# Ulixes-8/UNet-Implementations

Hardware: AMD Instinct MI355X
Metric: images/sec (512x512, bs/GPU=8) Our_UNet train step (higher is better)
Workload: dtype f32

## Files before the change

### unet-implementations_amd/csrc/conv_wino.hip

```cpp
#include "conv_params.h"
#include "lds_asm.h"
#include <utility>

namespace unet_conv {
namespace {

typedef int i32x4v __attribute__((ext_vector_type(4)));
template <int I> using wn_ic = std::integral_constant<int, I>;
template <int B, int... I, typename F>
__device__ __forceinline__ void wn_for_impl(std::integer_sequence<int, I...>, F&& f) {
  (f(wn_ic<B + I>{}), ...);
}
template <int B, int E, typename F>
__device__ __forceinline__ void wn_for(F&& f) {
  wn_for_impl<B>(std::make_integer_sequence<int, E - B>{}, f);
}

constexpr int WN_TH = 8, WN_TW = 32;
constexpr int WN_PW = WN_TW + 2, WN_PH = WN_TH + 2;
constexpr int WN_PPIX = WN_PH * WN_PW;
constexpr int WN_BN = 64;
constexpr int WN_KC = 8;
constexpr int WN_RP = 360;
constexpr int WN_BUF = 16 * 64 * WN_KC;
constexpr size_t WN_LDS = (size_t)(4 * WN_BUF + 2 * WN_KC * WN_RP) * sizeof(float);

__host__ __device__ __forceinline__ int wn_swz(int row, int k) {
  return 2 * ((k >> 1) ^ ((row >> 2) & 3)) + (k & 1);
}

struct WinoParams {
  IgemmParams g;
  const float* wu;
};

template <bool ACT, bool STATS, bool BSTATS, bool UP = false>
__global__ __launch_bounds__(512, 2) void conv_wino_kernel(const WinoParams wp) {
  const IgemmParams& p = wp.g;
  extern __shared__ __attribute__((aligned(16))) float smem[];
  float* Vs = smem;
  float* Us = smem + 2 * WN_BUF;
  float* Rs = smem + 4 * WN_BUF;

  const int tid = threadIdx.x, lane = tid & 63, wave = tid >> 6;
  const int H = p.Hin, W = p.Win;
  const int tiles_n = p.Ncols / WN_BN, tiles_x = W / WN_TW, tiles_y = H / WN_TH;
  int bid = xcd_remap(blockIdx.x, gridDim.x);
  const int tn = bid % tiles_n; bid /= tiles_n;
  const int tx = bid % tiles_x; bid /= tiles_x;
  const int ty = bid % tiles_y;
  const int n = bid / tiles_y;
  const int y0 = ty * WN_TH, x0 = tx * WN_TW, n0 = tn * WN_BN;
  const int Ktot = p.C0 + p.C1;
  const int chunks = Ktot / WN_KC;

  const __amdgpu_buffer_rsrc_t rs0 = __builtin_amdgcn_make_buffer_rsrc(
      const_cast<float*>(p.src0), 0, (int)p.src0_bytes, 0x00020000);
  const __amdgpu_buffer_rsrc_t rs1 = __builtin_amdgcn_make_buffer_rsrc(
      const_cast<float*>(p.src1 ? p.src1 : p.src0), 0, (int)p.src1_bytes, 0x00020000);

  const int half = tid & 1;
  unsigned voff0[UP ? 1 : 2], voff1[2];
  bool okslot[2];
#pragma unroll
  for (int i = 0; i < 2; ++i) {
    const int slot = tid + 512 * i;
    const int pix = slot >> 1;
    const int prow = pix / WN_PW, pcol = pix - prow * WN_PW;
    const int iy = y0 - 1 + prow, ix = x0 - 1 + pcol;
    const bool ok = slot < 2 * WN_PPIX && (unsigned)iy < (unsigned)H && (unsigned)ix < (unsigned)W;
    const unsigned lin = (unsigned)((n * H + iy) * W + ix);
    okslot[i] = ok;
    if (!UP) voff0[i] = ok ? (lin * (unsigned)p.C0 + half * 4) * 4u : 0x80000000u;
    voff1[i] = ok ? (lin * (unsigned)p.C1 + half * 4) * 4u : 0x80000000u;
  }
  int l_lin[2], l_meta[2];
  const int lw = W >> 1;
  if (UP) {
    const int h = H >> 1, w = W >> 1;
#pragma unroll
    for (int i = 0; i < 2; ++i) {
      const int slot = tid + 512 * i;
      const int pix = slot < 2 * WN_PPIX ? slot >> 1 : 0;
      const int prow = pix / WN_PW, pcol = pix - prow * WN_PW;
      int gy0 = (y0 >> 1) - 1 + (prow >> 1), gx0 = (x0 >> 1) - 1 + (pcol >> 1);
      int gy1 = gy0 + 1, gx1 = gx0 + 1;
      gy0 = gy0 < 0 ? 0 : (gy0 > h - 1 ? h - 1 : gy0);
      gy1 = gy1 < 0 ? 0 : (gy1 > h - 1 ? h - 1 : gy1);
      gx0 = gx0 < 0 ? 0 : (gx0 > w - 1 ? w - 1 : gx0);
      gx1 = gx1 < 0 ? 0 : (gx1 > w - 1 ? w - 1 : gx1);
      l_lin[i] = (n * h + gy0) * w + gx0;
      l_meta[i] = (gx1 - gx0) | ((gy1 - gy0) << 1) | ((pcol & 1) << 2) | ((prow & 1) << 3);
    }
  }
  constexpr int NSET = UP ? 1 : 2;
  f32x4 pr[NSET][2];
  f32x4 pt[UP ? 2 : 1][3];
  bool pup = false;
  f32x4 ca[NSET], cb[NSET];
#pragma unroll
  for (int q = 0; q < NSET; ++q) { ca[q] = f32x4{1.f, 1.f, 1.f, 1.f}; cb[q] = f32x4{0.f, 0.f, 0.f, 0.f}; }
  const unsigned hoff = (unsigned)half * 16u;
  auto load_raw = [&](int chunk, auto ic, auto setc) {
    constexpr int i = decltype(ic)::value;
    constexpr int Q = decltype(setc)::value;
    const int c = chunk * WN_KC;
    const bool first = c < p.C0;
    const __amdgpu_buffer_rsrc_t rs = first ? rs0 : rs1;
    const int Cs = first ? p.C0 : p.C1;
    const int cc = first ? c : c - p.C0;
    if (UP && first) {
      if (i == 1) pup = true;
      const unsigned o = (unsigned)(l_lin[i] * Cs + cc + half * 4);
      const unsigned dx = (l_meta[i] & 1) ? (unsigned)Cs : 0u;
      const unsigned dy = (l_meta[i] & 2) ? (unsigned)(lw * Cs) : 0u;
      pr[Q][i] = buf_ld4<float>(rs, o, 0u);
      if constexpr (UP) {
        pt[i][0] = buf_ld4<float>(rs, o + dx, 0u);
        pt[i][1] = buf_ld4<float>(rs, o + dy, 0u);
        pt[i][2] = buf_ld4<float>(rs, o + dy + dx, 0u);
      }
    } else {
      if (UP && i == 1) pup = false;
      unsigned vo = voff1[i];
      if constexpr (!UP) vo = first ? voff0[i] : voff1[i];
      pr[Q][i] = __builtin_bit_cast(f32x4, __builtin_amdgcn_raw_buffer_load_b128(rs, vo, cc * 4, 0));
    }
    if (ACT && i == 1) {
      const float* al = (first ? p.act0_alpha : p.act1_alpha) + ((size_t)n * Cs + cc);
      const float* be = (first ? p.act0_beta : p.act1_beta) + ((size_t)n * Cs + cc);
      ca[Q] = *reinterpret_cast<const f32x4*>(reinterpret_cast<const char*>(al) + hoff);
      cb[Q] = *reinterpret_cast<const f32x4*>(reinterpret_cast<const char*>(be) + hoff);
    }
  };
  const int rpix1 = tid < 2 * WN_PPIX - 512 ? 256 + (tid >> 1) : WN_PPIX + (tid & 15);
  float* const rdst0 = Rs + (half * 4) * WN_RP + (tid >> 1);
  float* const rdst1 = Rs + (half * 4) * WN_RP + rpix1;
  constexpr int RB = WN_KC * WN_RP;
#pragma unroll
  for (int i = 0; i < 2; ++i)
    if (!okslot[i] && tid + 512 * i < 2 * WN_PPIX) {
      float* d = i == 0 ? rdst0 : rdst1;
#pragma unroll
      for (int k = 0; k < 4; ++k) d[k * WN_RP] = d[RB + k * WN_RP] = 0.f;
    }
  auto store_raw = [&](auto ic, auto bc, auto setc) {
    constexpr int i = decltype(ic)::value;
    constexpr int B = decltype(bc)::value;
    constexpr int Q = decltype(setc)::value;
    f32x4 v = pr[Q][i];
    if (ACT) {
      const f32x4 a1 = ca[Q], b1 = cb[Q];
      const float sl = p.slope;
      bool done = false;
      if constexpr (UP) {
        if (pup) {
          const f32x4 p00 = act4f(v, a1, b1, sl, 1.f), p01 = act4f(pt[i][0], a1, b1, sl, 1.f);
          const f32x4 p10 = act4f(pt[i][1], a1, b1, sl, 1.f);
          const f32x4 p11 = act4f(pt[i][2], a1, b1, sl, 1.f);
          const float wx1 = (l_meta[i] & 4) ? 0.75f : 0.25f, wx0 = 1.f - wx1;
          const float wy1 = (l_meta[i] & 8) ? 0.75f : 0.25f, wy0 = 1.f - wy1;
          v = (p00 * wx0 + p01 * wx1) * wy0 + (p10 * wx0 + p11 * wx1) * wy1;
          done = true;
        }
      }
      if (!done) v = act4f(v, a1, b1, sl, 1.f);
    }
    if (okslot[i]) {
      float* d = (i == 0 ? rdst0 : rdst1) + B * RB;
      d[0] = v[0]; d[WN_RP] = v[1]; d[2 * WN_RP] = v[2]; d[3 * WN_RP] = v[3];
    }
  };
  const int t_tile = tid >> 3, t_ch = tid & 7;
  const unsigned t_ra = lds_addr(Rs + t_ch * WN_RP + (2 * (t_tile >> 4)) * WN_PW + 2 * (t_tile & 15));
  float* const t_vdst = Vs + t_tile * 8 + wn_swz(t_tile, t_ch);
  f32x2v tr[4];
  auto t_rd = [&](auto ac, auto bc) {
    constexpr int a = decltype(ac)::value;
    constexpr int B = decltype(bc)::value;
    constexpr int r0 = a == 0 ? 0 : (a == 1 ? 1 : (a == 2 ? 2 : 1));
    constexpr int r1 = a == 0 ? 2 : (a == 1 ? 2 : (a == 2 ? 1 : 3));
    tr[0] = lds_rd64<(B * RB + r0 * WN_PW) * 4>(t_ra);
    tr[1] = lds_rd64<(B * RB + r0 * WN_PW) * 4 + 8>(t_ra);
    tr[2] = lds_rd64<(B * RB + r1 * WN_PW) * 4>(t_ra);
    tr[3] = lds_rd64<(B * RB + r1 * WN_PW) * 4 + 8>(t_ra);
  };
  auto t_wr = [&](auto ac, auto bc) {
    constexpr int a = decltype(ac)::value;
    constexpr int B = decltype(bc)::value;
    lds_wait<15>(tr[0], tr[1], tr[2], tr[3]);
    const f32x2v lo = a == 1 ? tr[0] + tr[2] : tr[0] - tr[2];
    const f32x2v hi = a == 1 ? tr[1] + tr[3] : tr[1] - tr[3];
    float* Vb = t_vdst + B * WN_BUF;
    Vb[(4 * a + 0) * 512] = lo[0] - hi[0];
    Vb[(4 * a + 1) * 512] = lo[1] + hi[0];
    Vb[(4 * a + 2) * 512] = hi[0] - lo[1];
    Vb[(4 * a + 3) * 512] = lo[1] - hi[1];
  };
  const float* ubase = wp.wu + (size_t)((p.n_off / WN_BN + tn) * chunks) * WN_BUF;
  const int uwave = __builtin_amdgcn_readfirstlane(wave) * 1024;
  const unsigned lane16 = (unsigned)lane * 16u;
  const unsigned u_m0 = __builtin_amdgcn_readfirstlane(lds_addr(Us + uwave));
  auto dma_u = [&](int chunk, auto bc, auto ic) {
    constexpr int i = decltype(ic)::value;
    constexpr int B = decltype(bc)::value;
    const float* src = ubase + (size_t)chunk * WN_BUF + uwave;
    const unsigned m0v = u_m0 + B * WN_BUF * 4;
    dma16_sbase<i * 1024>(m0v, lane16, src);
  };

  const int tg = wave & 3, nh = wave >> 2;
  const int fm = lane & 15, fk = lane >> 4;
  const int fsw = 2 * (fk ^ ((fm >> 2) & 3));
  const unsigned va = lds_addr(Vs + (16 * tg + fm) * 8 + fsw);
  const unsigned ub = lds_addr(Us + (32 * nh + fm) * 8 + fsw);
  f32x4 acc[16][2];
#pragma unroll
  for (int x = 0; x < 16; ++x)
#pragma unroll
    for (int b = 0; b < 2; ++b) acc[x][b] = f32x4{0.f, 0.f, 0.f, 0.f};
  constexpr int FS = UP ? 1 : 2;
  f32x2v fa[FS], fb0[FS], fb1[FS];
  auto frag = [&](auto bc, auto xc) {
    constexpr int x = decltype(xc)::value;
    constexpr int B = decltype(bc)::value;
    constexpr int sl = x % FS;
    fa[sl] = lds_rd64<(B * WN_BUF + x * 512) * 4>(va);
    fb0[sl] = lds_rd64<(B * WN_BUF + x * 512) * 4>(ub);
    fb1[sl] = lds_rd64<(B * WN_BUF + x * 512 + 128) * 4>(ub);
  };
  auto mm = [&](auto xc) {
    constexpr int x = decltype(xc)::value;
    constexpr int sl = x % FS;
    acc[x][0] = __builtin_amdgcn_mfma_f32_16x16x4f32(fa[sl][0], fb0[sl][0], acc[x][0], 0, 0, 0);
    acc[x][1] = __builtin_amdgcn_mfma_f32_16x16x4f32(fa[sl][0], fb1[sl][0], acc[x][1], 0, 0, 0);
    acc[x][0] = __builtin_amdgcn_mfma_f32_16x16x4f32(fa[sl][1], fb0[sl][1], acc[x][0], 0, 0, 0);
    acc[x][1] = __builtin_amdgcn_mfma_f32_16x16x4f32(fa[sl][1], fb1[sl][1], acc[x][1], 0, 0, 0);
  };
  auto stage = [&](auto bc, auto xc, auto trc) {
    constexpr int x = decltype(xc)::value;
    constexpr int TR = decltype(trc)::value;
    constexpr int sl = x % FS;
    if constexpr (FS == 2) {
      if constexpr (x + 1 < 16) frag(bc, wn_ic<x + 1>{});
      lds_wait<(x + 1 < 16 ? 3 : 0) + TR>(fa[sl], fb0[sl], fb1[sl]);
      __builtin_amdgcn_sched_barrier(0);
      mm(xc);
    } else {
      lds_wait<0>(fa[sl], fb0[sl], fb1[sl]);
      __builtin_amdgcn_sched_barrier(0);
      mm(xc);
      if constexpr (x + 1 < 16) frag(bc, wn_ic<x + 1>{});
    }
  };

  using S0 = wn_ic<0>;
  using S1 = wn_ic<NSET - 1>;
  auto cl = [&](int c) { return c < chunks ? c : chunks - 1; };
  auto vm_done = [&]() {
    asm volatile("s_waitcnt vmcnt(0)" ::: "memory");
#pragma unroll
    for (int q = 0; q < NSET; ++q) reg_anchor(ca[q], cb[q]);
  };
  if constexpr (NSET == 2) {
    load_raw(0, wn_ic<0>{}, S0{});
    load_raw(0, wn_ic<1>{}, S0{});
    load_raw(cl(1), wn_ic<0>{}, S1{});
    load_raw(cl(1), wn_ic<1>{}, S1{});
    wn_for<0, 4>([&](auto ic) { dma_u(0, wn_ic<0>{}, ic); });
    vm_done();
    store_raw(wn_ic<0>{}, wn_ic<0>{}, S0{});
    store_raw(wn_ic<1>{}, wn_ic<0>{}, S0{});
    store_raw(wn_ic<0>{}, wn_ic<1>{}, S1{});
    store_raw(wn_ic<1>{}, wn_ic<1>{}, S1{});
    load_raw(cl(2), wn_ic<0>{}, S0{});
    load_raw(cl(2), wn_ic<1>{}, S0{});
    load_raw(cl(3), wn_ic<0>{}, S1{});
    load_raw(cl(3), wn_ic<1>{}, S1{});
    __syncthreads();
    wn_for<0, 4>([&](auto ac) {
      t_rd(ac, wn_ic<0>{});
      asm volatile("s_waitcnt lgkmcnt(0)" ::: "memory");
      t_wr(ac, wn_ic<0>{});
    });
  } else {
    load_raw(0, wn_ic<0>{}, S0{});
    load_raw(0, wn_ic<1>{}, S0{});
    wn_for<0, 4>([&](auto ic) { dma_u(0, wn_ic<0>{}, ic); });
    vm_done();
    store_raw(wn_ic<0>{}, wn_ic<0>{}, S0{});
    store_raw(wn_ic<1>{}, wn_ic<0>{}, S0{});
    load_raw(cl(1), wn_ic<0>{}, S0{});
    load_raw(cl(1), wn_ic<1>{}, S0{});
    __syncthreads();
    wn_for<0, 4>([&](auto ac) {
      t_rd(ac, wn_ic<0>{});
      asm volatile("s_waitcnt lgkmcnt(0)" ::: "memory");
      t_wr(ac, wn_ic<0>{});
    });
    vm_done();
    store_raw(wn_ic<0>{}, wn_ic<1>{}, S0{});
    store_raw(wn_ic<1>{}, wn_ic<1>{}, S0{});
    load_raw(cl(2), wn_ic<0>{}, S0{});
    load_raw(cl(2), wn_ic<1>{}, S0{});
  }
  auto chunk_body = [&](int c, auto bc) {
    constexpr int B = decltype(bc)::value;
    using NB = wn_ic<B ^ 1>;
    using SB = wn_ic<(NSET == 2 ? B : 0)>;
    if constexpr (NSET == 2) {
      if constexpr (ACT) asm volatile("s_waitcnt vmcnt(4) lgkmcnt(0)" ::: "memory");
      else asm volatile("s_waitcnt vmcnt(2) lgkmcnt(0)" ::: "memory");
    } else {
      asm volatile("s_waitcnt vmcnt(0) lgkmcnt(0)" ::: "memory");
    }
    __builtin_amdgcn_s_barrier();
    reg_anchor(ca[SB::value], cb[SB::value]);
    frag(bc, wn_ic<0>{});
    wn_for<0, 16>([&](auto xc) {
      constexpr int x = decltype(xc)::value;
      if constexpr (FS == 2) {
        constexpr bool T = x >= 8 && x < 12;
        if constexpr (T) t_rd(wn_ic<(T ? x - 8 : 0)>{}, NB{});
        stage(bc, xc, wn_ic<(T ? 4 : 0)>{});
        if constexpr (T) {
          lds_wait<3>(tr[0], tr[1], tr[2], tr[3]);
          t_wr(wn_ic<(T ? x - 8 : 0)>{}, NB{});
        }
      } else {
        stage(bc, xc, wn_ic<0>{});
        if constexpr (x >= 8 && x < 12) t_wr(wn_ic<(x >= 8 && x < 12 ? x - 8 : 0)>{}, NB{});
        if constexpr (x >= 7 && x < 11) t_rd(wn_ic<(x >= 7 && x < 11 ? x - 7 : 0)>{}, NB{});
      }
      if constexpr (NSET == 2) {
        if constexpr (x == 0) store_raw(wn_ic<0>{}, bc, SB{});
        if constexpr (x == 1) store_raw(wn_ic<1>{}, bc, SB{});
        if constexpr (x >= 2 && x < 6) dma_u(cl(c + 1), NB{}, wn_ic<(x >= 2 && x < 6 ? x - 2 : 0)>{});
        if constexpr (x == 6) load_raw(cl(c + 4), wn_ic<0>{}, SB{});
        if constexpr (x == 7) load_raw(cl(c + 4), wn_ic<1>{}, SB{});
      } else {
        if constexpr (x == 0) store_raw(wn_ic<0>{}, bc, SB{});
        if constexpr (x == 1) load_raw(cl(c + 3), wn_ic<0>{}, SB{});
        if constexpr (x == 2) store_raw(wn_ic<1>{}, bc, SB{});
        if constexpr (x == 3) load_raw(cl(c + 3), wn_ic<1>{}, SB{});
        if constexpr (x >= 4 && x < 8) dma_u(cl(c + 1), NB{}, wn_ic<(x >= 4 && x < 8 ? x - 4 : 0)>{});
      }
      __builtin_amdgcn_sched_barrier(0);
    });
  };
  for (int c = 0; c < chunks; c += 2) {
    chunk_body(c, wn_ic<0>{});
    if (c + 1 < chunks) chunk_body(c + 1, wn_ic<1>{});
  }

  int etid = threadIdx.x;
  asm volatile("" : "+v"(etid));
  const int fm_e = etid & 15, fk_e = (etid >> 4) & 3, tg_e = (etid >> 6) & 3, nh_e = etid >> 8;
  float yv[2][4][4];
#pragma unroll
  for (int b = 0; b < 2; ++b) {
    const int col = n0 + 32 * nh_e + 16 * b + fm_e;
    const float bv = p.bias ? p.bias[p.n_off + col] : 0.f;
#pragma unroll
    for (int r = 0; r < 4; ++r) {
      float s[4][2];
#pragma unroll
      for (int i = 0; i < 4; ++i) {
        s[i][0] = acc[4 * i + 0][b][r] + acc[4 * i + 1][b][r] + acc[4 * i + 2][b][r];
        s[i][1] = acc[4 * i + 1][b][r] - acc[4 * i + 2][b][r] - acc[4 * i + 3][b][r];
      }
#pragma unroll
      for (int j = 0; j < 2; ++j) {
        yv[b][r][j] = s[0][j] + s[1][j] + s[2][j] + bv;
        yv[b][r][2 + j] = s[1][j] - s[2][j] - s[3][j] + bv;
      }
    }
  }
  const int oy = y0 + 2 * tg_e, ox = x0 + 2 * (4 * fk_e);
#pragma unroll
  for (int b = 0; b < 2; ++b) {
    const int col = n0 + 32 * nh_e + 16 * b + fm_e;
#pragma unroll
    for (int r = 0; r < 4; ++r)
#pragma unroll
      for (int q = 0; q < 4; ++q) {
        const size_t pix = ((size_t)n * H + oy + (q >> 1)) * W + ox + 2 * r + (q & 1);
        p.out[pix * p.ldo + col] = yv[b][r][q];
      }
  }
  float2* red = reinterpret_cast<float2*>(Rs);
  if (STATS && p.stats) {
    __syncthreads();
#pragma unroll
    for (int b = 0; b < 2; ++b) {
      float sm = 0.f;
#pragma unroll
      for (int r = 0; r < 4; ++r)
#pragma unroll
        for (int q = 0; q < 4; ++q) sm += yv[b][r][q];
      float mean = sm * (1.f / 16.f), m2 = 0.f;
#pragma unroll
      for (int r = 0; r < 4; ++r)
#pragma unroll
        for (int q = 0; q < 4; ++q) {
          const float d = yv[b][r][q] - mean;
          m2 = fmaf(d, d, m2);
        }
      wf_merge_eq(mean, m2, __shfl_xor(mean, 16, 64), __shfl_xor(m2, 16, 64), 16.f);
      wf_merge_eq(mean, m2, __shfl_xor(mean, 32, 64), __shfl_xor(m2, 32, 64), 32.f);
      if (fk_e == 0) red[tg_e * WN_BN + 32 * nh_e + 16 * b + fm_e] = float2{mean, m2};
    }
    float2 out;
    if (block_col_stats<WN_BN, 4>(red, 0, 0, false, float2{0.f, 0.f}, 64.f, out))
      p.stats[((size_t)n * p.stats_tiles + ty * tiles_x + tx) * p.Ncols + n0 + tid] = out;
  }
  if (BSTATS && p.bs_partial) {
    __syncthreads();
#pragma unroll
    for (int b = 0; b < 2; ++b) {
      const int col = n0 + 32 * nh_e + 16 * b + fm_e;
      const BwdCoef cf = bwd_coef(p, n, col);
      float s1 = 0.f, s2 = 0.f;
#pragma unroll
      for (int r = 0; r < 4; ++r)
#pragma unroll
        for (int q = 0; q < 4; ++q) {
          const size_t pix = ((size_t)n * H + oy + (q >> 1)) * W + ox + 2 * r + (q & 1);
          const float y = p.bs_y[pix * p.ldo + col];
          const float z = fmaf(y, cf.A, cf.B0);
          const float gz = yv[b][r][q] * cf.mk * (z > 0.f ? 1.f : p.slope);
          s1 += gz;
          s2 = fmaf(gz, (y - cf.mu) * cf.rs, s2);
        }
      s1 += __shfl_xor(s1, 16, 64); s2 += __shfl_xor(s2, 16, 64);
      s1 += __shfl_xor(s1, 32, 64); s2 += __shfl_xor(s2, 32, 64);
      if (fk_e == 0) red[tg_e * WN_BN + 32 * nh_e + 16 * b + fm_e] = float2{s1, s2};
    }
    float2 out;
    if (block_col_sums<WN_BN, 4>(red, out))
      p.bs_partial[((size_t)n * p.bs_tiles + ty * tiles_x + tx) * p.Ncols + n0 + tid] = out;
  }
}

__device__ __forceinline__ void wino_pack_items(const float* __restrict__ w,
                                                float* __restrict__ uf, float* __restrict__ ud,
                                                int Cout, int Cin, int dir, long long block) {
  float* dst = dir == 0 ? uf : ud;
  if (!dst) return;
  const int Nn = dir == 0 ? Cout : Cin, Kt = dir == 0 ? Cin : Cout;
  const int kchunks = Kt / WN_KC;
  const long long items = (long long)Nn * kchunks;
  const long long idx = block * 256 + threadIdx.x;
  if (idx >= items) return;
  const int nl = (int)(idx & 63);
  const long long rest = idx >> 6;
  const int kc = (int)(rest % kchunks), tn = (int)(rest / kchunks);
  const int nn = tn * WN_BN + nl;
  float u[16][8];
#pragma unroll
  for (int k = 0; k < 8; ++k) {
    const int kk = kc * WN_KC + k;
    const int co = dir == 0 ? nn : kk, ci = dir == 0 ? kk : nn;
    const float* g = w + ((size_t)co * Cin + ci) * 9;
    float t4[4][3];
#pragma unroll
    for (int v = 0; v < 3; ++v) {
      const float g0 = dir == 0 ? g[0 + v] : g[6 + 2 - v];
      const float g1 = dir == 0 ? g[3 + v] : g[3 + 2 - v];
      const float g2 = dir == 0 ? g[6 + v] : g[0 + 2 - v];
      t4[0][v] = g0;
      t4[1][v] = 0.5f * (g0 + g1 + g2);
      t4[2][v] = 0.5f * (g0 - g1 + g2);
      t4[3][v] = g2;
    }
#pragma unroll
    for (int a = 0; a < 4; ++a) {
      u[4 * a + 0][k] = t4[a][0];
      u[4 * a + 1][k] = 0.5f * (t4[a][0] + t4[a][1] + t4[a][2]);
      u[4 * a + 2][k] = 0.5f * (t4[a][0] - t4[a][1] + t4[a][2]);
      u[4 * a + 3][k] = t4[a][2];
    }
  }
  const bool s1 = (nl >> 2) & 1, s2 = (nl >> 3) & 1;
  float* blk = dst + ((size_t)tn * kchunks + kc) * WN_BUF + nl * 8;
#pragma unroll
  for (int x = 0; x < 16; ++x) {
    f32x2v p0 = {u[x][0], u[x][1]}, p1 = {u[x][2], u[x][3]}, p2 = {u[x][4], u[x][5]},
           p3 = {u[x][6], u[x][7]};
    const f32x2v q0 = s1 ? p1 : p0, q1 = s1 ? p0 : p1, q2 = s1 ? p3 : p2, q3 = s1 ? p2 : p3;
    p0 = s2 ? q2 : q0; p1 = s2 ? q3 : q1; p2 = s2 ? q0 : q2; p3 = s2 ? q1 : q3;
    *reinterpret_cast<f32x4*>(blk + x * 512) = f32x4{p0[0], p0[1], p1[0], p1[1]};
    *reinterpret_cast<f32x4*>(blk + x * 512 + 4) = f32x4{p2[0], p2[1], p3[0], p3[1]};
  }
}

__global__ __launch_bounds__(256) void wino_pack_kernel(const float* __restrict__ w,
                                                        float* __restrict__ uf,
                                                        float* __restrict__ ud, int Cout, int Cin) {
  wino_pack_items(w, uf, ud, Cout, Cin, blockIdx.y, blockIdx.x);
}
__global__ __launch_bounds__(256) void wino_pack_batched_kernel(
    const unet_wino_pack_entry* __restrict__ tab, int n) {
  int k = 0;
  for (int q = 1; q < n; ++q)
    if (tab[q].block_begin <= (int)blockIdx.x) k = q;
  const unet_wino_pack_entry e = tab[k];
  wino_pack_items(e.w, e.uf, e.ud, e.Cout, e.Cin, blockIdx.y, (long long)blockIdx.x - e.block_begin);
}

template <bool ACT, bool STATS, bool BSTATS, bool UP = false>
int launch_wino(const WinoParams& wp, hipStream_t stream) {
  auto kern = conv_wino_kernel<ACT, STATS, BSTATS, UP>;
  UNET_SET_DYN_LDS(kern, WN_LDS);
  const IgemmParams& p = wp.g;
  const long long tiles =
      (long long)p.N * (p.Hin / WN_TH) * (p.Win / WN_TW) * (p.Ncols / WN_BN);
  const long long blocks = tiles;
  hipLaunchKernelGGL(kern, dim3((unsigned)blocks), dim3(512), WN_LDS, stream, wp);
  UNET_CHECK_LAUNCH("conv_wino");
  return UNET_OK;
}

bool wino_shape_ok(int N, int H, int W, int K0, int K1, int ncols, int n_off, bool up = false) {
  const int K = K0 + K1;
  if (H % WN_TH || W % WN_TW || K0 % WN_KC || K1 % WN_KC || ncols % WN_BN || n_off % WN_BN)
    return false;
  if (K < 64 || (up && K0 < WN_KC)) return false;
  const long long px = (long long)N * H * W;
  const long long b0 = (up ? px / 4 : px) * K0 * 4, b1 = px * K1 * 4;
  if (b0 >= (1LL << 31) || b1 >= (1LL << 31) || px * ncols * 4 >= (1LL << 31)) return false;
  return px / (WN_TH * WN_TW) * (ncols / WN_BN) >= 256;
}

}
}

using namespace unet_conv;

extern "C" int unet_conv_wino_supported(int N, int H, int W, int C0, int C1, int Cout) {
  return wino_shape_ok(N, H, W, C0, C1, Cout, 0) ? 1 : 0;
}

extern "C" int unet_conv_up_wino_supported(int N, int H, int W, int C0, int C1, int Cout) {
  return wino_shape_ok(N, H, W, C0, C1, Cout, 0, true) ? 1 : 0;
}

extern "C" size_t unet_wino_weight_floats(int Cout, int Cin) { return (size_t)16 * Cout * Cin; }

extern "C" int unet_pack_wino_weights(const float* w_oihw, float* uf, float* ud, int Cout, int Cin,
                                      unet_stream_t stream) {
  UNET_REQUIRE(w_oihw && (uf || ud) && Cout > 0 && Cin > 0, "pack_wino_weights: bad argument");
  UNET_REQUIRE(!uf || (Cout % WN_BN == 0 && Cin % WN_KC == 0),
               "pack_wino_weights: forward form needs Cout %% 64 == 0, Cin %% 8 == 0");
  UNET_REQUIRE(!ud || (Cin % WN_BN == 0 && Cout % WN_KC == 0),
               "pack_wino_weights: data-gradient form needs Cin %% 64 == 0, Cout %% 8 == 0");
  const long long items = (long long)Cout * Cin / WN_KC;
  hipLaunchKernelGGL(wino_pack_kernel, dim3((unsigned)((items + 255) / 256), 2), dim3(256), 0,
                     (hipStream_t)stream, w_oihw, uf, ud, Cout, Cin);
  UNET_CHECK_LAUNCH("wino_pack");
  return UNET_OK;
}

extern "C" int unet_pack_wino_weights_batched(const unet_wino_pack_entry* table_device, int n,
                                              int total_blocks, unet_stream_t stream) {
  UNET_REQUIRE(table_device && n > 0 && n <= 256 && total_blocks > 0,
               "pack_wino_weights_batched: bad argument");
  hipLaunchKernelGGL(wino_pack_batched_kernel, dim3((unsigned)total_blocks, 2), dim3(256), 0,
                     (hipStream_t)stream, table_device, n);
  UNET_CHECK_LAUNCH("wino_pack_batched");
  return UNET_OK;
}

static int conv_in_fwd_wino_impl(const unet_act_src* s0, const unet_act_src* s1, float slope,
                                 const float* wu, const float* bias, float* y, void* workspace,
                                 size_t workspace_bytes, int* stats_px_out, int N, int H, int W,
                                 int Cout, hipStream_t stream, bool up) {
  UNET_REQUIRE(s0 && s0->x && wu && y && stats_px_out, "conv_in_fwd_wino: null pointer");
  const int C0 = s0->C, C1 = s1 ? s1->C : 0;
  UNET_REQUIRE(C1 == 0 || s1->x, "conv_in_fwd_wino: second source is null with C1=%d", C1);
  UNET_REQUIRE(s0->alpha && s0->beta && (!s1 || (s1->alpha && s1->beta)),
               "conv_in_fwd_wino: the Winograd loader takes activated sources (alpha / beta set)");
  UNET_REQUIRE(wino_shape_ok(N, H, W, C0, C1, Cout, 0, up),
               "conv_in_fwd_wino: shape N=%d %dx%d C=(%d,%d)->%d not tiled by the Winograd kernel",
               N, H, W, C0, C1, Cout);
  UNET_REQUIRE(!up || (H % 2 == 0 && W % 2 == 0 && C1 > 0), "conv_up_in_fwd_wino: bad shape");
  const int tiles = H * W / 256;
  const size_t need = (size_t)N * tiles * Cout * sizeof(float2);
  if (workspace && workspace_bytes < need) {
    unet_set_error("conv_in_fwd_wino: workspace %zu < %zu bytes", workspace_bytes, need);
    return UNET_E_WORKSPACE;
  }
  WinoParams wp{};
  IgemmParams& p = wp.g;
  p.src0 = s0->x; p.src1 = s1 ? s1->x : nullptr; p.C0 = C0; p.C1 = C1;
  p.act0_alpha = s0->alpha; p.act0_beta = s0->beta;
  p.act1_alpha = s1 ? s1->alpha : nullptr;
  p.act1_beta = s1 ? s1->beta : nullptr;
  p.slope = slope;
  p.src0_bytes = (unsigned)((long long)N * (up ? H / 2 : H) * (up ? W / 2 : W) * C0 * 4);
  p.src1_bytes = (unsigned)((long long)N * H * W * C1 * 4);
  p.bias = bias; p.n_off = 0;
  p.out = y; p.ldo = Cout; p.N = N; p.Hin = p.Hl = p.Hout = H; p.Win = p.Wl = p.Wout = W;
  p.Ncols = Cout;
  p.stats = reinterpret_cast<float2*>(workspace);
  p.stats_tiles = tiles;
  wp.wu = wu;
  *stats_px_out = workspace ? 256 : 0;
  if (up) return launch_wino<true, true, false, true>(wp, stream);
  return launch_wino<true, true, false>(wp, stream);
}

extern "C" int unet_conv_in_fwd_wino(const unet_act_src* s0, const unet_act_src* s1, float slope,
                                     const float* wu, const float* bias, float* y, void* workspace,
                                     size_t workspace_bytes, int* stats_px_out, int N, int H,
                                     int W, int Cout, unet_stream_t stream) {
  return conv_in_fwd_wino_impl(s0, s1, slope, wu, bias, y, workspace, workspace_bytes,
                               stats_px_out, N, H, W, Cout, (hipStream_t)stream, false);
}

extern "C" int unet_conv_up_in_fwd_wino(const unet_act_src* low, const unet_act_src* skip,
                                        float slope, const float* wu, const float* bias, float* y,
                                        void* workspace, size_t workspace_bytes,
                                        int* stats_px_out, int N, int H, int W, int Cout,
                                        unet_stream_t stream) {
  return conv_in_fwd_wino_impl(low, skip, slope, wu, bias, y, workspace, workspace_bytes,
                               stats_px_out, N, H, W, Cout, (hipStream_t)stream, true);
}

extern "C" int unet_conv3x3_bwd_data_bs_wino(const float* dy, const float* ud, int Cin_total,
                                             int ci_offset, float* dx, int N, int H, int W,
                                             int Cout, int Ccols, unet_bwd_stats* bs,
                                             unet_stream_t stream) {
  UNET_REQUIRE(dy && ud && dx, "conv3x3_bwd_data_bs_wino: null pointer");
  UNET_REQUIRE(ci_offset >= 0 && ci_offset + Ccols <= Cin_total && Cin_total % WN_BN == 0,
               "conv3x3_bwd_data_bs_wino: bad channel slice");
  UNET_REQUIRE(wino_shape_ok(N, H, W, Cout, 0, Ccols, ci_offset),
               "conv3x3_bwd_data_bs_wino: shape N=%d %dx%d %d->%d not tiled by the Winograd kernel",
               N, H, W, Cout, Ccols);
  WinoParams wp{};
  IgemmParams& p = wp.g;
  p.src0 = dy; p.C0 = Cout; p.C1 = 0;
  p.src0_bytes = (unsigned)((long long)N * H * W * Cout * 4);
  p.n_off = ci_offset;
  p.out = dx; p.ldo = Ccols; p.N = N; p.Hin = p.Hl = p.Hout = H; p.Win = p.Wl = p.Wout = W;
  p.Ncols = Ccols;
  wp.wu = ud;
  const bool use_bs = bs && bs->y && bs->mean && bs->rstd && bs->gamma && bs->beta &&
                      bs->partial &&
                      bs->partial_bytes >= (size_t)N * (H * W / 256) * Ccols * sizeof(float2);
  if (bs) bs->tiles_out = 0;
  if (use_bs) {
    p.bs_y = bs->y; p.bs_mean = bs->mean; p.bs_rstd = bs->rstd; p.bs_gamma = bs->gamma;
    p.bs_beta = bs->beta; p.bs_mask = bs->mask; p.slope = bs->slope;
    p.bs_partial = reinterpret_cast<float2*>(bs->partial);
    p.bs_tiles = H * W / 256; p.bs_tile0 = 0;
    bs->tiles_out = p.bs_tiles;
    return launch_wino<false, false, true>(wp, (hipStream_t)stream);
  }
  return launch_wino<false, false, false>(wp, (hipStream_t)stream);
}
```

Measured before the change: 468.0.

## Stage low-res upsample tile in LDS and fuse bilinear into Winograd input transform

For the fused-upsample Winograd conv, each thread previously issued four global loads per padded pixel and interpolated in registers. Now the kernel loads each low-resolution pixel once into a new LDS staging region, then computes the bilinear upsample while doing the Winograd input transform from a 3x3 neighbourhood. This also lets the UP variant use the same double-buffered raw pipeline (NSET=2, FS=2) as the non-UP path. In exchange it uses more LDS per block and needs extra border-padding logic plus tighter waitcnt handling.

Result: no change. 468.8 (median of 6 runs) (+0.2%).

```diff
diff --git a/unet-implementations_amd/csrc/conv_wino.hip b/unet-implementations_amd/csrc/conv_wino.hip
--- a/unet-implementations_amd/csrc/conv_wino.hip
+++ b/unet-implementations_amd/csrc/conv_wino.hip
@@ -24,7 +24,25 @@
 constexpr int WN_RP = 360;
 constexpr int WN_BUF = 16 * 64 * WN_KC;
 constexpr size_t WN_LDS = (size_t)(4 * WN_BUF + 2 * WN_KC * WN_RP) * sizeof(float);
-
+constexpr int WN_LH = WN_TH / 2 + 2, WN_LW = WN_TW / 2 + 2;
+constexpr int WN_LSLOTS = 2 * WN_LH * WN_LW;
+constexpr int WN_LB = WN_LH * WN_LW * WN_KC;
+constexpr size_t WN_LDS_UP = WN_LDS + (size_t)2 * WN_LB * sizeof(float);
+static_assert(8 * 27 == WN_LSLOTS && WN_LDS_UP <= 160 * 1024, "UP staging: 27 slots per wave");
+
+template <int OFF>
+__device__ __forceinline__ float lds_rd32(unsigned a) {
+  float v;
+  asm volatile("ds_read_b32 %0, %1 offset:%2" : "=v"(v) : "v"(a), "n"(OFF) : "memory");
+  return v;
+}
+template <int N>
+__device__ __forceinline__ void lds_wait9(float (&l)[9]) {
+  asm volatile("s_waitcnt lgkmcnt(%9)"
+               : "+v"(l[0]), "+v"(l[1]), "+v"(l[2]), "+v"(l[3]), "+v"(l[4]), "+v"(l[5]),
+                 "+v"(l[6]), "+v"(l[7]), "+v"(l[8])
+               : "n"(N));
+}
 __host__ __device__ __forceinline__ int wn_swz(int row, int k) {
   return 2 * ((k >> 1) ^ ((row >> 2) & 3)) + (k & 1);
 }
@@ -41,6 +59,7 @@
   float* Vs = smem;
   float* Us = smem + 2 * WN_BUF;
   float* Rs = smem + 4 * WN_BUF;
+  float* Ls = Rs + 2 * WN_KC * WN_RP;
 
   const int tid = threadIdx.x, lane = tid & 63, wave = tid >> 6;
   const int H = p.Hin, W = p.Win;
@@ -74,29 +93,24 @@
     if (!UP) voff0[i] = ok ? (lin * (unsigned)p.C0 + half * 4) * 4u : 0x80000000u;
     voff1[i] = ok ? (lin * (unsigned)p.C1 + half * 4) * 4u : 0x80000000u;
   }
-  int l_lin[2], l_meta[2];
-  const int lw = W >> 1;
-  if (UP) {
+  unsigned l_off = 0x80000000u;
+  bool l_ok = false;
+  float* l_dst = Ls;
+  if constexpr (UP) {
     const int h = H >> 1, w = W >> 1;
-#pragma unroll
-    for (int i = 0; i < 2; ++i) {
-      const int slot = tid + 512 * i;
-      const int pix = slot < 2 * WN_PPIX ? slot >> 1 : 0;
-      const int prow = pix / WN_PW, pcol = pix - prow * WN_PW;
-      int gy0 = (y0 >> 1) - 1 + (prow >> 1), gx0 = (x0 >> 1) - 1 + (pcol >> 1);
-      int gy1 = gy0 + 1, gx1 = gx0 + 1;
-      gy0 = gy0 < 0 ? 0 : (gy0 > h - 1 ? h - 1 : gy0);
-      gy1 = gy1 < 0 ? 0 : (gy1 > h - 1 ? h - 1 : gy1);
-      gx0 = gx0 < 0 ? 0 : (gx0 > w - 1 ? w - 1 : gx0);
-      gx1 = gx1 < 0 ? 0 : (gx1 > w - 1 ? w - 1 : gx1);
-      l_lin[i] = (n * h + gy0) * w + gx0;
-      l_meta[i] = (gx1 - gx0) | ((gy1 - gy0) << 1) | ((pcol & 1) << 2) | ((prow & 1) << 3);
-    }
-  }
-  constexpr int NSET = UP ? 1 : 2;
+    const int slot = wave * 27 + lane - (wave & 1);
+    l_ok = lane >= (wave & 1) && lane < 27 + (wave & 1);
+    const int pix = l_ok ? slot >> 1 : 0;
+    const int lr = pix / WN_LW, lc = pix - lr * WN_LW;
+    int gy = (y0 >> 1) - 1 + lr, gx = (x0 >> 1) - 1 + lc;
+    gy = gy < 0 ? 0 : (gy > h - 1 ? h - 1 : gy);
+    gx = gx < 0 ? 0 : (gx > w - 1 ? w - 1 : gx);
+    if (l_ok) l_off = ((unsigned)((n * h + gy) * w + gx) * (unsigned)p.C0 + half * 4) * 4u;
+    l_dst = Ls + (l_ok ? slot : 0) * 4;
+  }
+  constexpr int NSET = 2;
   f32x4 pr[NSET][2];
-  f32x4 pt[UP ? 2 : 1][3];
-  bool pup = false;
+  bool pup[NSET] = {false, false};
   f32x4 ca[NSET], cb[NSET];
 #pragma unroll
   for (int q = 0; q < NSET; ++q) { ca[q] = f32x4{1.f, 1.f, 1.f, 1.f}; cb[q] = f32x4{0.f, 0.f, 0.f, 0.f}; }
@@ -109,23 +123,13 @@
     const __amdgpu_buffer_rsrc_t rs = first ? rs0 : rs1;
     const int Cs = first ? p.C0 : p.C1;
     const int cc = first ? c : c - p.C0;
-    if (UP && first) {
-      if (i == 1) pup = true;
-      const unsigned o = (unsigned)(l_lin[i] * Cs + cc + half * 4);
-      const unsigned dx = (l_meta[i] & 1) ? (unsigned)Cs : 0u;
-      const unsigned dy = (l_meta[i] & 2) ? (unsigned)(lw * Cs) : 0u;
-      pr[Q][i] = buf_ld4<float>(rs, o, 0u);
-      if constexpr (UP) {
-        pt[i][0] = buf_ld4<float>(rs, o + dx, 0u);
-        pt[i][1] = buf_ld4<float>(rs, o + dy, 0u);
-        pt[i][2] = buf_ld4<float>(rs, o + dy + dx, 0u);
-      }
-    } else {
-      if (UP && i == 1) pup = false;
-      unsigned vo = voff1[i];
-      if constexpr (!UP) vo = first ? voff0[i] : voff1[i];
-      pr[Q][i] = __builtin_bit_cast(f32x4, __builtin_amdgcn_raw_buffer_load_b128(rs, vo, cc * 4, 0));
-    }
+    unsigned vo = voff1[i];
+    if constexpr (!UP) vo = first ? voff0[i] : voff1[i];
+    else {
+      if (i == 0) pup[Q] = first;
+      if (first) vo = i == 0 ? l_off : 0x80000000u;
+    }
+    pr[Q][i] = __builtin_bit_cast(f32x4, __builtin_amdgcn_raw_buffer_load_b128(rs, vo, cc * 4, 0));
     if (ACT && i == 1) {
       const float* al = (first ? p.act0_alpha : p.act1_alpha) + ((size_t)n * Cs + cc);
       const float* be = (first ? p.act0_beta : p.act1_beta) + ((size_t)n * Cs + cc);
@@ -149,22 +153,12 @@
     constexpr int B = decltype(bc)::value;
     constexpr int Q = decltype(setc)::value;
     f32x4 v = pr[Q][i];
-    if (ACT) {
-      const f32x4 a1 = ca[Q], b1 = cb[Q];
-      const float sl = p.slope;
-      bool done = false;
-      if constexpr (UP) {
-        if (pup) {
-          const f32x4 p00 = act4f(v, a1, b1, sl, 1.f), p01 = act4f(pt[i][0], a1, b1, sl, 1.f);
-          const f32x4 p10 = act4f(pt[i][1], a1, b1, sl, 1.f);
-          const f32x4 p11 = act4f(pt[i][2], a1, b1, sl, 1.f);
-          const float wx1 = (l_meta[i] & 4) ? 0.75f : 0.25f, wx0 = 1.f - wx1;
-          const float wy1 = (l_meta[i] & 8) ? 0.75f : 0.25f, wy0 = 1.f - wy1;
-          v = (p00 * wx0 + p01 * wx1) * wy0 + (p10 * wx0 + p11 * wx1) * wy1;
-          done = true;
-        }
+    if (ACT) v = act4f(v, ca[Q], cb[Q], p.slope, 1.f);
+    if constexpr (UP) {
+      if (pup[Q]) {
+        if (i == 0 && l_ok) *reinterpret_cast<f32x4*>(l_dst + B * WN_LB) = v;
+        return;
       }
-      if (!done) v = act4f(v, a1, b1, sl, 1.f);
     }
     if (okslot[i]) {
       float* d = (i == 0 ? rdst0 : rdst1) + B * RB;
@@ -197,6 +191,63 @@
     Vb[(4 * a + 2) * 512] = hi[0] - lo[1];
     Vb[(4 * a + 3) * 512] = lo[1] - hi[1];
   };
+  float tl[9];
+  unsigned t_la = 0;
+  bool wg_border = false, p_top = false, p_bot = false, p_lft = false, p_rgt = false;
+  if constexpr (UP) {
+    const int ty_t = t_tile >> 4, tx_t = t_tile & 15;
+    t_la = lds_addr(Ls + (ty_t * WN_LW + tx_t) * WN_KC + t_ch);
+    wg_border = y0 == 0 || y0 + WN_TH == H || x0 == 0 || x0 + WN_TW == W;
+    p_top = y0 == 0 && ty_t == 0;
+    p_bot = y0 + WN_TH == H && ty_t == 3;
+    p_lft = x0 == 0 && tx_t == 0;
+    p_rgt = x0 + WN_TW == W && tx_t == 15;
+  }
+  auto tu_rd = [&](auto bc) {
+    constexpr int B = decltype(bc)::value;
+    wn_for<0, 9>([&](auto ic) {
+      constexpr int r = decltype(ic)::value / 3, c = decltype(ic)::value % 3;
+      tl[3 * r + c] = lds_rd32<(B * WN_LB + (r * WN_LW + c) * WN_KC) * 4>(t_la);
+    });
+  };
+  auto tu_wr_impl = [&](auto bc, auto pc) {
+    constexpr bool PAD = decltype(pc)::value;
+    float cb4[3][4];
+#pragma unroll
+    for (int r = 0; r < 3; ++r)
+#pragma unroll
+      for (int m = 0; m < 4; ++m) {
+        const float w1 = (m & 1) ? 0.75f : 0.25f, w0 = 1.f - w1;
+        cb4[r][m] = fmaf(tl[3 * r + (m >> 1) + 1], w1, tl[3 * r + (m >> 1)] * w0);
+      }
+    float d[4][4];
+#pragma unroll
+    for (int k = 0; k < 4; ++k)
+#pragma unroll
+      for (int m = 0; m < 4; ++m) {
+        const float w1 = (k & 1) ? 0.75f : 0.25f, w0 = 1.f - w1;
+        d[k][m] = fmaf(w0, cb4[k >> 1][m], w1 * cb4[(k >> 1) + 1][m]);
+        if constexpr (PAD) {
+          const bool pad = (k == 0 && p_top) || (k == 3 && p_bot) || (m == 0 && p_lft) ||
+                           (m == 3 && p_rgt);
+          d[k][m] = pad ? 0.f : d[k][m];
+        }
+      }
+    wn_for<0, 4>([&](auto ac) {
+      constexpr int a = decltype(ac)::value;
+      constexpr int r0 = a == 0 ? 0 : (a == 1 ? 1 : (a == 2 ? 2 : 1));
+      constexpr int r1 = a == 0 ? 2 : (a == 1 ? 2 : (a == 2 ? 1 : 3));
+      tr[0] = f32x2v{d[r0][0], d[r0][1]};
+      tr[1] = f32x2v{d[r0][2], d[r0][3]};
+      tr[2] = f32x2v{d[r1][0], d[r1][1]};
+      tr[3] = f32x2v{d[r1][2], d[r1][3]};
+      t_wr(ac, bc);
+    });
+  };
+  auto tu_wr = [&](auto bc) {
+    if (wg_border) tu_wr_impl(bc, std::true_type{});
+    else tu_wr_impl(bc, std::false_type{});
+  };
   const float* ubase = wp.wu + (size_t)((p.n_off / WN_BN + tn) * chunks) * WN_BUF;
   const int uwave = __builtin_amdgcn_readfirstlane(wave) * 1024;
   const unsigned lane16 = (unsigned)lane * 16u;
@@ -219,7 +270,7 @@
   for (int x = 0; x < 16; ++x)
 #pragma unroll
     for (int b = 0; b < 2; ++b) acc[x][b] = f32x4{0.f, 0.f, 0.f, 0.f};
-  constexpr int FS = UP ? 1 : 2;
+  constexpr int FS = 2;
   f32x2v fa[FS], fb0[FS], fb1[FS];
   auto frag = [&](auto bc, auto xc) {
     constexpr int x = decltype(xc)::value;
@@ -241,110 +292,89 @@
     constexpr int x = decltype(xc)::value;
     constexpr int TR = decltype(trc)::value;
     constexpr int sl = x % FS;
-    if constexpr (FS == 2) {
-      if constexpr (x + 1 < 16) frag(bc, wn_ic<x + 1>{});
-      lds_wait<(x + 1 < 16 ? 3 : 0) + TR>(fa[sl], fb0[sl], fb1[sl]);
-      __builtin_amdgcn_sched_barrier(0);
-      mm(xc);
-    } else {
-      lds_wait<0>(fa[sl], fb0[sl], fb1[sl]);
-      __builtin_amdgcn_sched_barrier(0);
-      mm(xc);
-      if constexpr (x + 1 < 16) frag(bc, wn_ic<x + 1>{});
-    }
+    if constexpr (x + 1 < 16) frag(bc, wn_ic<x + 1>{});
+    lds_wait<(x + 1 < 16 ? 3 : 0) + TR>(fa[sl], fb0[sl], fb1[sl]);
+    __builtin_amdgcn_sched_barrier(0);
+    mm(xc);
   };
 
   using S0 = wn_ic<0>;
-  using S1 = wn_ic<NSET - 1>;
+  using S1 = wn_ic<1>;
   auto cl = [&](int c) { return c < chunks ? c : chunks - 1; };
   auto vm_done = [&]() {
     asm volatile("s_waitcnt vmcnt(0)" ::: "memory");
 #pragma unroll
     for (int q = 0; q < NSET; ++q) reg_anchor(ca[q], cb[q]);
   };
-  if constexpr (NSET == 2) {
-    load_raw(0, wn_ic<0>{}, S0{});
-    load_raw(0, wn_ic<1>{}, S0{});
-    load_raw(cl(1), wn_ic<0>{}, S1{});
-    load_raw(cl(1), wn_ic<1>{}, S1{});
-    wn_for<0, 4>([&](auto ic) { dma_u(0, wn_ic<0>{}, ic); });
-    vm_done();
-    store_raw(wn_ic<0>{}, wn_ic<0>{}, S0{});
-    store_raw(wn_ic<1>{}, wn_ic<0>{}, S0{});
-    store_raw(wn_ic<0>{}, wn_ic<1>{}, S1{});
-    store_raw(wn_ic<1>{}, wn_ic<1>{}, S1{});
-    load_raw(cl(2), wn_ic<0>{}, S0{});
-    load_raw(cl(2), wn_ic<1>{}, S0{});
-    load_raw(cl(3), wn_ic<0>{}, S1{});
-    load_raw(cl(3), wn_ic<1>{}, S1{});
-    __syncthreads();
+  load_raw(0, wn_ic<0>{}, S0{});
+  load_raw(0, wn_ic<1>{}, S0{});
+  load_raw(cl(1), wn_ic<0>{}, S1{});
+  load_raw(cl(1), wn_ic<1>{}, S1{});
+  wn_for<0, 4>([&](auto ic) { dma_u(0, wn_ic<0>{}, ic); });
+  vm_done();
+  store_raw(wn_ic<0>{}, wn_ic<0>{}, S0{});
+  store_raw(wn_ic<1>{}, wn_ic<0>{}, S0{});
+  store_raw(wn_ic<0>{}, wn_ic<1>{}, S1{});
+  store_raw(wn_ic<1>{}, wn_ic<1>{}, S1{});
+  load_raw(cl(2), wn_ic<0>{}, S0{});
+  load_raw(cl(2), wn_ic<1>{}, S0{});
+  load_raw(cl(3), wn_ic<0>{}, S1{});
+  load_raw(cl(3), wn_ic<1>{}, S1{});
+  __syncthreads();
+  if constexpr (UP) {
+    tu_rd(wn_ic<0>{});
+    lds_wait9<0>(tl);
+    tu_wr(wn_ic<0>{});
+  } else {
     wn_for<0, 4>([&](auto ac) {
       t_rd(ac, wn_ic<0>{});
       asm volatile("s_waitcnt lgkmcnt(0)" ::: "memory");
       t_wr(ac, wn_ic<0>{});
     });
-  } else {
-    load_raw(0, wn_ic<0>{}, S0{});
-    load_raw(0, wn_ic<1>{}, S0{});
-    wn_for<0, 4>([&](auto ic) { dma_u(0, wn_ic<0>{}, ic); });
-    vm_done();
-    store_raw(wn_ic<0>{}, wn_ic<0>{}, S0{});
-    store_raw(wn_ic<1>{}, wn_ic<0>{}, S0{});
-    load_raw(cl(1), wn_ic<0>{}, S0{});
-    load_raw(cl(1), wn_ic<1>{}, S0{});
-    __syncthreads();
-    wn_for<0, 4>([&](auto ac) {
-      t_rd(ac, wn_ic<0>{});
-      asm volatile("s_waitcnt lgkmcnt(0)" ::: "memory");
-      t_wr(ac, wn_ic<0>{});
-    });
-    vm_done();
-    store_raw(wn_ic<0>{}, wn_ic<1>{}, S0{});
-    store_raw(wn_ic<1>{}, wn_ic<1>{}, S0{});
-    load_raw(cl(2), wn_ic<0>{}, S0{});
-    load_raw(cl(2), wn_ic<1>{}, S0{});
   }
   auto chunk_body = [&](int c, auto bc) {
     constexpr int B = decltype(bc)::value;
     using NB = wn_ic<B ^ 1>;
-    using SB = wn_ic<(NSET == 2 ? B : 0)>;
-    if constexpr (NSET == 2) {
-      if constexpr (ACT) asm volatile("s_waitcnt vmcnt(4) lgkmcnt(0)" ::: "memory");
-      else asm volatile("s_waitcnt vmcnt(2) lgkmcnt(0)" ::: "memory");
-    } else {
-      asm volatile("s_waitcnt vmcnt(0) lgkmcnt(0)" ::: "memory");
-    }
+    using SB = wn_ic<B>;
+    if constexpr (ACT) asm volatile("s_waitcnt vmcnt(4) lgkmcnt(0)" ::: "memory");
+    else asm volatile("s_waitcnt vmcnt(2) lgkmcnt(0)" ::: "memory");
     __builtin_amdgcn_s_barrier();
     reg_anchor(ca[SB::value], cb[SB::value]);
     frag(bc, wn_ic<0>{});
+    const bool up_next = UP && (c + 1) * WN_KC < p.C0;
     wn_for<0, 16>([&](auto xc) {
       constexpr int x = decltype(xc)::value;
-      if constexpr (FS == 2) {
-        constexpr bool T = x >= 8 && x < 12;
+      constexpr bool T = x >= 8 && x < 12;
+      if constexpr (UP && (T || x == 7)) {
+        if constexpr (x == 7) {
+          tu_rd(NB{});
+          stage(bc, xc, wn_ic<9>{});
+        } else {
+          constexpr int sn = (x + 1) % FS;
+          t_rd(wn_ic<x - 8>{}, NB{});
+          stage(bc, xc, wn_ic<4>{});
+          lds_wait<0>(tr[0], tr[1], tr[2], tr[3]);
+          if constexpr (x + 1 < 16) lds_wait<0>(fa[sn], fb0[sn], fb1[sn]);
+          if constexpr (x == 8) lds_wait9<0>(tl);
+          if (up_next) {
+            if constexpr (x == 8) tu_wr(NB{});
+          } else {
+            t_wr(wn_ic<x - 8>{}, NB{});
+          }
+        }
+      } else {
         if constexpr (T) t_rd(wn_ic<(T ? x - 8 : 0)>{}, NB{});
         stage(bc, xc, wn_ic<(T ? 4 : 0)>{});
         if constexpr (T) {
           lds_wait<3>(tr[0], tr[1], tr[2], tr[3]);
           t_wr(wn_ic<(T ? x - 8 : 0)>{}, NB{});
         }
-      } else {
-        stage(bc, xc, wn_ic<0>{});
-        if constexpr (x >= 8 && x < 12) t_wr(wn_ic<(x >= 8 && x < 12 ? x - 8 : 0)>{}, NB{});
-        if constexpr (x >= 7 && x < 11) t_rd(wn_ic<(x >= 7 && x < 11 ? x - 7 : 0)>{}, NB{});
       }
-      if constexpr (NSET == 2) {
-        if constexpr (x == 0) store_raw(wn_ic<0>{}, bc, SB{});
-        if constexpr (x == 1) store_raw(wn_ic<1>{}, bc, SB{});
-        if constexpr (x >= 2 && x < 6) dma_u(cl(c + 1), NB{}, wn_ic<(x >= 2 && x < 6 ? x - 2 : 0)>{});
-        if constexpr (x == 6) load_raw(cl(c + 4), wn_ic<0>{}, SB{});
-        if constexpr (x == 7) load_raw(cl(c + 4), wn_ic<1>{}, SB{});
-      } else {
-        if constexpr (x == 0) store_raw(wn_ic<0>{}, bc, SB{});
-        if constexpr (x == 1) load_raw(cl(c + 3), wn_ic<0>{}, SB{});
-        if constexpr (x == 2) store_raw(wn_ic<1>{}, bc, SB{});
-        if constexpr (x == 3) load_raw(cl(c + 3), wn_ic<1>{}, SB{});
-        if constexpr (x >= 4 && x < 8) dma_u(cl(c + 1), NB{}, wn_ic<(x >= 4 && x < 8 ? x - 4 : 0)>{});
-      }
+      if constexpr (x == 0) store_raw(wn_ic<0>{}, bc, SB{});
+      if constexpr (x == 1) store_raw(wn_ic<1>{}, bc, SB{});
+      if constexpr (x >= 2 && x < 6) dma_u(cl(c + 1), NB{}, wn_ic<(x >= 2 && x < 6 ? x - 2 : 0)>{});
+      if constexpr (x == 6) load_raw(cl(c + 4), wn_ic<0>{}, SB{});
+      if constexpr (x == 7) load_raw(cl(c + 4), wn_ic<1>{}, SB{});
       __builtin_amdgcn_sched_barrier(0);
     });
   };
@@ -511,12 +541,13 @@
 template <bool ACT, bool STATS, bool BSTATS, bool UP = false>
 int launch_wino(const WinoParams& wp, hipStream_t stream) {
   auto kern = conv_wino_kernel<ACT, STATS, BSTATS, UP>;
-  UNET_SET_DYN_LDS(kern, WN_LDS);
+  constexpr size_t lds = UP ? WN_LDS_UP : WN_LDS;
+  UNET_SET_DYN_LDS(kern, lds);
   const IgemmParams& p = wp.g;
   const long long tiles =
       (long long)p.N * (p.Hin / WN_TH) * (p.Win / WN_TW) * (p.Ncols / WN_BN);
   const long long blocks = tiles;
-  hipLaunchKernelGGL(kern, dim3((unsigned)blocks), dim3(512), WN_LDS, stream, wp);
+  hipLaunchKernelGGL(kern, dim3((unsigned)blocks), dim3(512), lds, stream, wp);
   UNET_CHECK_LAUNCH("conv_wino");
   return UNET_OK;
 }
```
